# Ex10si0n/room-slam

Measured on NVIDIA B200. Metric: train traces/sec (seq500, H128) at 1/2/4/8 B200; heatmap Gpoints/s, higher is better.
Workload: dtype bf16

## Files before the change

include/roomslam_b200.h:

```cpp
#ifndef ROOMSLAM_B200_H
#define ROOMSLAM_B200_H

#include <stdint.h>

#ifdef __cplusplus
extern "C" {
#endif

const char* rs_last_error(void);
int rs_abi_version(void);
int rs_device_ok(void);
int64_t rs_launch_count(void);
int rs_set_deterministic(int on);
int rs_deterministic(void);

int rs_heatmap_bin(const float* points, int64_t n_traces, int64_t seq_len, float x_min, float y_min, float res,
                   int gx, int gy, float thr2, int32_t* occ, int32_t* stat, unsigned long long* n_dropped,
                   int accumulate, void* stream);
int rs_heatmap_bin_variant(const float* points, int64_t n_traces, int64_t seq_len, float x_min, float y_min,
                           float res, int gx, int gy, float thr2, int32_t* occ, int32_t* stat,
                           unsigned long long* n_dropped, int accumulate, int variant, void* stream);
int rs_heatmap_bin_host(const float* host_points, int64_t n_traces, int64_t seq_len, float x_min, float y_min,
                        float res, int gx, int gy, float thr2, int32_t* host_occ, int32_t* host_stat,
                        unsigned long long* host_dropped);

#define RS_GEMM_ACCUMULATE 1
#define RS_GEMM_RELU 2
#define RS_GEMM_OUT_F32 4
int rs_sgemm(const float* A, int64_t a_sm, int64_t a_sk, const float* B, int64_t b_sk, int64_t b_sn, float* C,
             int64_t ldc, const float* bias, int M, int N, int K, int flags, void* stream);
int rs_colsum_f32(const float* A, int64_t lda, int M, int N, float* out, int accumulate, void* stream);
int rs_gru_fwd_f32(const float* x, int64_t x_ld, int64_t x_rows, int64_t x_row0, int I, const float* w_ih,
                   const float* b_ih, const float* P, int64_t p_ld, int64_t p_rows, int64_t p_row0,
                   const float* w_hh_t, const float* b_hh, float* out, int64_t o_ld, int64_t o_rows, int64_t o_row0,
                   float* h_n, float* gates, const int* lengths, int B, int T, int H, void* stream);
int rs_gru_bwd_f32(const float* d_out, int64_t do_ld, int64_t do_rows, int64_t do_row0, const float* d_h_n,
                   const float* gates, const float* out, int64_t o_ld, int64_t o_rows, int64_t o_row0,
                   const float* w_hh, float* dGx, float* dGh, int64_t g_ld, int64_t g_rows, int64_t g_row0,
                   const int* lengths, int B, int T, int H, void* stream);
int rs_seq_mul_f32(const float* a, int64_t a_ld, int64_t a_rows, int64_t a_row0, const float* m, int64_t m_ld,
                   int64_t m_rows, int64_t m_row0, float* o, int64_t o_ld, int64_t o_rows, int64_t o_row0, int B, int T,
                   int C, void* stream);
int rs_heads_split_f32(const float* raw, int B, int N, int C, float* cls, float* pos, float* size, float* orient,
                       float* valid, void* stream);
int rs_heads_merge_bwd_f32(const float* raw, int B, int N, int C, const float* d_cls, const float* d_pos,
                           const float* d_size, const float* d_orient, const float* d_valid, float* d_raw, void* stream);
int rs_relu_bwd_f32(const float* dy, const float* y, float* dx, int64_t n, void* stream);
int rs_relu_bwd_bf16(const void* dy, const void* y, void* dx, int64_t n, void* stream);
int rs_loss_fwd_f32(const float* cls, const float* pos, const float* size, const float* orient, const float* vlogit,
                    const int64_t* t_cls, const float* t_pos, const float* t_size, const float* t_orient,
                    const float* t_valid, int B, int N, int C, const float* weights5, double* sums6, float* losses6,
                    float* g_cls, float* g_pos, float* g_size, float* g_orient, float* g_valid, void* stream);
int rs_loss_bwd_f32(const double* sums6, const float* d_losses6, int B, int N, int C, const float* weights5,
                    const float* g_cls, const float* g_pos, const float* g_size, const float* g_orient,
                    const float* g_valid, float* d_cls, float* d_pos, float* d_size, float* d_orient, float* d_valid,
                    void* stream);

int rs_gemm_bf16_nt(const void* A, int64_t lda, const void* B, int64_t ldb, void* C, int64_t ldc, const float* bias,
                    int64_t M, int N, int K, int flags, void* stream);
int rs_gemm_bf16_tn_acc(const void* A, int64_t lda, int64_t a_rows, int a_col0, int a_row_shift, const void* B,
                        int64_t ldb, int64_t b_rows, int b_col0, int b_row_shift, float* C, int64_t ldc, int M, int N,
                        int64_t rows, void* stream);

int rs_split_bf16x6(const float* x, int64_t ld, int64_t rows, int cols, int kpad, int role_b, void* out, int64_t ld_out,
                    void* stream);

int rs_gemm_bf16_tn_seg_acc(const void* A, int64_t lda, int64_t a_rows, int a_col0, int a_row_shift, const void* B,
                            int64_t ldb, int64_t b_rows, int b_col0, int b_row_shift, int n_seg, const int* a_seg,
                            const int* b_seg, float* C, int64_t ldc, int M, int N, int64_t rows, void* stream);

int rs_adamw_step_f32(float* p, const float* g, float* m, float* v, int64_t n, float lr, float beta1, float beta2,
                      float eps, float weight_decay, int step, float grad_scale, float max_norm, double* sumsq_scratch,
                      void* stream);

int rs_blk_gemm_nt(const void* A, int64_t a_cols, const int* a_kchunk, int k_blocks, const void* W, int n_tiles, void* C,
                   int64_t c_cols, int c_chunk0, const float* bias, int64_t n_blocks, void* stream);
int rs_blk_gemm_nt_drop(const void* A, int64_t a_cols, const int* a_kchunk, int k_blocks, const void* W, int n_tiles, void* C,
                        int64_t c_cols, int c_chunk0, int64_t n_blocks, const void* drop_bits, const float* drop_scale, int T,
                        void* stream);
int rs_blk_gemm_tn_acc(const void* A, int64_t a_cols, const int* a_mchunk, const int* c_row0, int m_tiles, const void* B,
                       int64_t b_cols, int b_chunk0, int n_cols, int b_shift, int b_broadcast, float* C, int64_t ldc,
                       int tiles, int T, void* stream);
int rs_blk_wgrad(const void* dG, int64_t a_cols, const void* ones_block, int n_roles, const int* a_mchunk,
                 const void* const* B, const int64_t* b_cols, const int* b_chunk0, const int* n_cols, const int* b_shift,
                 float* const* C, const int64_t* ldc, float* const* bias, const void* const* B2, float* const* C2,
                 int tiles, int T, void* stream);
int rs_gru_pack_weights_bf16(const float* const* w, int H, int I, int split, void* whh_img, float* b_hn, float* bias_x,
                             void* wt_proj, void* whhT_img, void* wt_dgrad, void* wih_img, void* stream);
int rs_rec_fwd_bf16(const float* x, int I, const void* P, int64_t p_cols, const void* X, const void* Wih, const void* Whh,
                    const float* b_hn, void* out,
                    void* gates, float* h_n, const int* lengths, const void* drop_bits, const float* drop_scale,
                    void* out_drop, int split, int B, int T, void* stream);
int rs_pack_x_tm(const float* x, int B, int T, int I, void* out, void* stream);
int rs_rec_bwd_bf16(const void* d_out, const float* d_h_n, const void* gates, const void* out, const void* WhhT,
                    const void* Whh, int whh_chunks, const float* b_hn, void* dG, const int* lengths, const void* drop_bits,
                    const float* drop_scale, int split, int B, int T, void* stream);
int rs_rec_fwd_bf16_wide(const float* x, int I, const void* P, const void* Wst, const float* b_hn, void* out, void* gates,
                         float* h_n, const int* lengths, const void* drop_bits, const float* drop_scale, void* out_drop,
                         int B, int T, void* stream);
int rs_rec_bwd_bf16_wide(const void* d_out, const float* d_h_n, const void* gates, const void* out, const void* WTst, void* dG,
                         const int* lengths, const void* drop_bits, const float* drop_scale, int B, int T, void* stream);
int rs_pack_drop_mask(const float* mask, int B, int T, int C, void* bits, float* scale, void* stream);
int rs_gen_drop_bits(void* bits, int B, int T, int C, float keep, uint64_t seed, float* scale, void* stream);

int rs_trace_features(const float* pts, const int64_t* offsets, int B, int max_len, int out_len, float* feats,
                      unsigned char* mask, int64_t* lengths, int* unsorted_flag, void* stream);

int rs_resample_windows_f64(const double* pts, const int64_t* offsets, const int64_t* win_trace, const int64_t* win_start,
                            int64_t n_windows, int seq_len, double step, float* out, void* stream);

int rs_lstm_fwd_f32(const float* P, int64_t p_ld, int64_t p_rows, int64_t p_row0, const float* w_hh, const float* w_hh_t,
                    float* out, int64_t o_ld, int64_t o_rows, int64_t o_row0, float* saved, int B, int T, int H,
                    void* stream);
int rs_lstm_bwd_f32(const float* d_out, int64_t do_ld, int64_t do_rows, int64_t do_row0, const float* saved,
                    const float* w_hh, float* dG, int64_t g_ld, int64_t g_rows, int64_t g_row0, int B, int T, int H,
                    void* stream);
int rs_trace_stats_f32(const float* traces, int F, const unsigned char* mask, int B, int N, float* mean, float* rms,
                       float* count, void* stream);
int64_t rs_query_attn_workspace(int B, int Q, int D, int splits);
int rs_query_attn_fwd_f32(const float* memory, int64_t m_ld, int64_t m_rows, int64_t m_row0, const float* traces, int F,
                          const unsigned char* mask, const float* mean, const float* rms, const float* qk, const float* qb,
                          int B, int N, int Q, int D, int splits, float* workspace, float* ctx, float* anchor,
                          float* summary, float* stats, void* stream);
int rs_query_attn_bwd_f32(const float* memory, int64_t m_ld, int64_t m_rows, int64_t m_row0, const float* traces, int F,
                          const unsigned char* mask, const float* mean, const float* rms, const float* count,
                          const float* qk, const float* qb, const float* ctx, const float* anchor, const float* stats,
                          const float* d_ctx, const float* d_anchor, const float* d_summary, int B, int N, int Q, int D,
                          int splits, float* d_memory, int64_t dm_ld, int64_t dm_rows, int64_t dm_row0, float* dq_part,
                          void* stream);

int rs_hungarian_match(const float* pred_boxes, const float* pred_logits, const float* gt_boxes, const int64_t* gt_labels,
                       const unsigned char* gt_valid, int B, int Q, int M, float w_class, float w_box, int* match_pred,
                       int* match_slot, int* match_rank, int* n_match, void* stream);
int rs_set_loss_f32(const float* pred_boxes, const float* pred_logits, const float* gt_boxes, const int64_t* gt_labels, int B,
                    int Q, int M, const int* match_pred, const int* match_slot, const int* n_match, float w_class, float w_l1,
                    float w_giou, float* workspace, float* losses, float* g_logits, float* g_l1, float* g_giou, void* stream);

int rs_eval_pairs(const float* pred_boxes, const float* pred_logits, const float* gt_boxes, const int64_t* gt_labels,
                  const unsigned char* gt_valid, int B, int Q, int M, const int* match_pred, const int* match_slot,
                  const int* n_match, float iou_thresh, double* workspace, double* counts, void* stream);
int rs_nms_3d(const float* pred_boxes, const float* pred_logits, int B, int Q, float conf_thr, float nms_thr, int* keep_idx,
              int* n_keep, float* conf, int* label, void* stream);
int rs_ap_flags(const float* pred_boxes, const float* pred_logits, const float* gt_boxes, const int64_t* gt_labels,
                const unsigned char* gt_valid, int B, int Q, int M, float iou_thr, int* flags, float* conf, int* label, int* n_gt,
                void* stream);

int rs_slot_eval(const float* class_logits, const float* positions, const float* sizes, const float* validity_logits,
                 const int64_t* t_classes, const float* t_positions, const float* t_sizes, const float* t_valid,
                 int64_t n_slots, int C, float iou_thr, float* conf, int* label, int* flag, int* n_gt, double* workspace,
                 double* counts, void* stream);

#ifdef __cplusplus
}
#endif
#endif
```

roomslam_b200/csrc/gemm_blk.cu:

```cuda
#include <stdlib.h>

#include "common.cuh"
#include "../../include/roomslam_b200.h"

namespace {

constexpr int CHUNK_BYTES = 2048;
constexpr int PIECE_BYTES = 8 * CHUNK_BYTES;
constexpr int NT_STAGES_MAX = 6;
constexpr int NT_MAX_KB = 24;
constexpr int NUM_THREADS = 192;

struct NtParams {
    const uint8_t* A;  long long a_block_bytes;  int a_kchunk[NT_MAX_KB];
    const uint8_t* W;
    uint8_t* C;        long long c_block_bytes;  int c_chunk0;
    const float* bias;
    int n_blocks, n_tiles, k_blocks;
    const uint8_t* drop_bits; const float* drop_scale; int drop_T; int drop_row_bytes;
};

constexpr int NT_THREADS = 320;
constexpr int NT_MAX_N = 1024;

// ... 69 lines not shown
                for (int kb = 0; kb < p.k_blocks; ++kb) {
                    rs::mbar_wait(&full_bar[stage], phase);
                    rs::tc_fence_after();
                    if (rs::elect_one()) {
                        const uint32_t ss = rs::smem_u32(stages + stage * kStageBytes);
                        const uint32_t sa = kResident ? rs::smem_u32(a_res + (ab * 4 + kb) * PIECE_BYTES) : ss;
                        const uint32_t sb = kResident ? ss : ss + PIECE_BYTES;
#pragma unroll
                        for (int k = 0; k < 4; ++k) {
                            const uint64_t da = rs::umma_desc_noswz(sa + k * 2 * CHUNK_BYTES, CHUNK_BYTES, 128);
                            const uint64_t db = rs::umma_desc_noswz(sb + k * 2 * CHUNK_BYTES, CHUNK_BYTES, 128);
                            rs::tc_mma_bf16(tmem_d, da, db, idesc, (kb | k) != 0);
                        }
                        rs::tc_commit(&empty_bar[stage]);
                        if (kb == p.k_blocks - 1) {
                            rs::tc_commit(&acc_full[acc]);
                            if (kResident && n == p.n_tiles - 1) rs::tc_commit(&a_empty[ab]);
                        }
                    }
                    __syncwarp();
                    if (++stage == NT_STAGES) { stage = 0; phase ^= 1; }
                }
                if (++acc == 2) { acc = 0; acc_phase ^= 1; }
            }
            if (kResident && ++ab == 2) { ab = 0; a_phase ^= 1; }
        }
    } else {
        const int q = warp & 3, row = q * 32 + lane;
        const int chalf = (warp - 2) >> 2;
        int acc = 0; uint32_t acc_phase = 0;
        const float dscale = p.drop_bits ? __ldg(p.drop_scale) : 1.0f;
        for (int m = blockIdx.x; m < p.n_blocks; m += gridDim.x) {
            uint8_t* cblk = p.C + (long long)m * p.c_block_bytes + row * 16;
            const uint8_t* drow = nullptr;
            if (p.drop_bits) {
                const int tp = m % (p.drop_T + 2);
                if (tp >= 1 && tp <= p.drop_T)
                    drow = p.drop_bits + (((long long)(m / (p.drop_T + 2)) * p.drop_T + (tp - 1)) * 128 + row) * p.drop_row_bytes;
            }
            for (int n = 0; n < p.n_tiles; ++n) {
                rs::mbar_wait(&acc_full[acc], acc_phase);
                rs::tc_fence_after();
                const uint32_t taddr = tmem_base + acc * 128 + chalf * 64 + (static_cast<uint32_t>(q * 32) << 16);
#pragma unroll
                for (int c0 = 0; c0 < 64; c0 += 32) {
                    uint32_t r[32];
                    rs::tmem_ld_32x32b_x32(taddr + c0, r);
                    uint32_t mbits = 0xffffffffu;
                    if (drow) mbits = __ldg(reinterpret_cast<const uint32_t*>(drow + p.c_chunk0 + n * 16 + chalf * 8 + c0 / 8));
                    rs::tmem_ld_wait();
                    if (drow) {
#pragma unroll
                        for (int e = 0; e < 32; ++e)
                            r[e] = ((mbits >> e) & 1u) ? __float_as_uint(__uint_as_float(r[e]) * dscale) : 0u;
                    }
                    const float* bs = bias_s + n * 128 + chalf * 64 + c0;
#pragma unroll
                    for (int j = 0; j < 4; ++j) {
                        uint32_t pk[4];
                        const float4 b0 = *reinterpret_cast<const float4*>(bs + 8 * j);
                        const float4 b1 = *reinterpret_cast<const float4*>(bs + 8 * j + 4);
                        const float bb[8] = {b0.x, b0.y, b0.z, b0.w, b1.x, b1.y, b1.z, b1.w};
#pragma unroll
                        for (int e = 0; e < 4; ++e) {
                            const float v0 = __uint_as_float(r[8 * j + 2 * e]) + bb[2 * e];
                            const float v1 = __uint_as_float(r[8 * j + 2 * e + 1]) + bb[2 * e + 1];
                            __nv_bfloat162 h2 = __floats2bfloat162_rn(v0, v1);
                            pk[e] = *reinterpret_cast<uint32_t*>(&h2);
                        }
                        const int chunk = p.c_chunk0 + n * 16 + chalf * 8 + c0 / 8 + j;
                        *reinterpret_cast<uint4*>(cblk + (long long)chunk * CHUNK_BYTES) = make_uint4(pk[0], pk[1], pk[2], pk[3]);
                    }
                }
                rs::tc_fence_before();
                __syncwarp();
                if (lane == 0) rs::mbar_arrive(&acc_empty[acc]);
                if (++acc == 2) { acc = 0; acc_phase ^= 1; }
            }
        }
    }
    rs::tc_fence_before();
    __syncthreads();
    if (warp == 1) rs::tmem_dealloc<256>(tmem_base);
}

constexpr int WRES_STAGES = 5;
__global__ void __launch_bounds__(NT_THREADS, 1) blk_gemm_nt_wres_kernel(const NtParams p, int n_parts) {
    extern __shared__ __align__(1024) uint8_t smem[];
    uint8_t* w_s = smem;
    uint8_t* stages = smem + p.k_blocks * 2 * PIECE_BYTES;
    float* bias_s = reinterpret_cast<float*>(stages + WRES_STAGES * PIECE_BYTES);
    uint64_t* bars = reinterpret_cast<uint64_t*>(bias_s + 256);
    uint64_t* full_bar = bars;
    uint64_t* empty_bar = bars + WRES_STAGES;
    uint64_t* acc_full = bars + 2 * WRES_STAGES;
    uint64_t* acc_empty = bars + 2 * WRES_STAGES + 2;
    uint64_t* w_full = bars + 2 * WRES_STAGES + 4;
    uint32_t* tmem_slot = reinterpret_cast<uint32_t*>(bars + 2 * WRES_STAGES + 5);
    const int warp = threadIdx.x >> 5, lane = threadIdx.x & 31;
    const int part = blockIdx.x % n_parts, group = blockIdx.x / n_parts, groups = gridDim.x / n_parts;

    if (warp == 0 && lane == 0) {
        for (int s = 0; s < WRES_STAGES; ++s) { rs::mbar_init(&full_bar[s], 1); rs::mbar_init(&empty_bar[s], 1); }
        for (int s = 0; s < 2; ++s) { rs::mbar_init(&acc_full[s], 1); rs::mbar_init(&acc_empty[s], 8); }
        rs::mbar_init(w_full, 1);
        rs::fence_mbar_init();
    }
    if (warp == 1) rs::tmem_alloc<512>(tmem_slot);
    for (int i = threadIdx.x; i < 256; i += NT_THREADS) bias_s[i] = p.bias ? p.bias[part * 256 + i] : 0.0f;
    rs::tc_fence_before();
    __syncthreads();
    rs::tc_fence_after();
    const uint32_t tmem_base = *tmem_slot;

    if (warp == 0) {
        if (rs::elect_one()) {
            rs::mbar_expect_tx(w_full, p.k_blocks * 2 * PIECE_BYTES);
            for (int kb = 0; kb < p.k_blocks; ++kb)
                for (int half = 0; half < 2; ++half) {
                    const uint8_t* src = p.W + ((long long)(part * 2 + half) * p.k_blocks + kb) * PIECE_BYTES;
                    for (int c = 0; c < 8; ++c)
                        rs::bulk_load(w_s + kb * 2 * PIECE_BYTES + c * 2 * CHUNK_BYTES + half * CHUNK_BYTES, src + c * CHUNK_BYTES,
                                      CHUNK_BYTES, w_full);
                }
            int stage = 0; uint32_t phase = 0;
            for (int m = group; m < p.n_blocks; m += groups) {
                const uint8_t* ablk = p.A + (long long)m * p.a_block_bytes;
                for (int kb = 0; kb < p.k_blocks; ++kb) {
                    rs::mbar_wait(&empty_bar[stage], phase ^ 1);
                    rs::mbar_expect_tx(&full_bar[stage], PIECE_BYTES);
                    rs::bulk_load(stages + stage * PIECE_BYTES, ablk + (long long)p.a_kchunk[kb] * CHUNK_BYTES, PIECE_BYTES, &full_bar[stage]);
                    if (++stage == WRES_STAGES) { stage = 0; phase ^= 1; }
                }
            }
        }
    } else if (warp == 1) {
        constexpr uint32_t idesc = rs::umma_idesc_bf16(128, 256, 0, 0);
        rs::mbar_wait(w_full, 0);
        rs::tc_fence_after();
        int stage = 0; uint32_t phase = 0; int acc = 0; uint32_t acc_phase = 0;
        const uint32_t w_addr = rs::smem_u32(w_s);
        for (int m = group; m < p.n_blocks; m += groups) {
            rs::mbar_wait(&acc_empty[acc], acc_phase ^ 1);
            rs::tc_fence_after();
            const uint32_t tmem_d = tmem_base + acc * 256;
            for (int kb = 0; kb < p.k_blocks; ++kb) {
                rs::mbar_wait(&full_bar[stage], phase);
                rs::tc_fence_after();
                if (rs::elect_one()) {
                    const uint32_t sa = rs::smem_u32(stages + stage * PIECE_BYTES);
                    const uint32_t sb = w_addr + kb * 2 * PIECE_BYTES;
#pragma unroll
                    for (int k = 0; k < 4; ++k) {
                        const uint64_t da = rs::umma_desc_noswz(sa + k * 2 * CHUNK_BYTES, CHUNK_BYTES, 128);
                        const uint64_t db = rs::umma_desc_noswz(sb + k * 2 * (2 * CHUNK_BYTES), 2 * CHUNK_BYTES, 128);
                        rs::tc_mma_bf16(tmem_d, da, db, idesc, (kb | k) != 0);
                    }
                    rs::tc_commit(&empty_bar[stage]);
                    if (kb == p.k_blocks - 1) rs::tc_commit(&acc_full[acc]);
                }
                __syncwarp();
                if (++stage == WRES_STAGES) { stage = 0; phase ^= 1; }
            }
            if (++acc == 2) { acc = 0; acc_phase ^= 1; }
        }
    } else {
// ... 292 lines not shown
        if (i1 > i0) acc_phase ^= 1;
        __syncthreads();
        rs::tc_fence_after();
    }
    rs::tc_fence_before();
    __syncthreads();
    if (p.paired) rs::cluster_sync_all();
    if (warp == 1) rs::tmem_dealloc<512>(tmem_base);
}

int g_sms = 0;
int num_sms() {
    if (g_sms == 0) {
        int dev = 0;
        cudaGetDevice(&dev);
        cudaDeviceGetAttribute(&g_sms, cudaDevAttrMultiProcessorCount, dev);
    }
    return g_sms;
}

}

static int blk_gemm_nt_impl(const void* A, int64_t a_cols, const int* a_kchunk, int k_blocks, const void* W,
                            int n_tiles, void* C, int64_t c_cols, int c_chunk0, const float* bias, int64_t n_blocks,
                            const void* drop_bits, const float* drop_scale, int drop_T, void* stream_) {
    cudaStream_t stream = static_cast<cudaStream_t>(stream_);
    if (rs::check_device_sm100()) return 3;
    if (n_blocks == 0) return 0;
    RS_REQUIRE(A && W && C && a_kchunk, "rs_blk_gemm_nt: null pointer");
    RS_REQUIRE(k_blocks >= 1 && k_blocks <= NT_MAX_KB && n_tiles >= 1, "rs_blk_gemm_nt: 1 <= k_blocks <= %d", NT_MAX_KB);
    RS_REQUIRE(a_cols % 8 == 0 && c_cols % 8 == 0 && n_blocks < (1ll << 31), "rs_blk_gemm_nt: bad shape");
    NtParams p = {};
    p.A = static_cast<const uint8_t*>(A); p.a_block_bytes = a_cols * 256;
    for (int i = 0; i < k_blocks; ++i) {
        RS_REQUIRE(a_kchunk[i] >= 0 && (a_kchunk[i] + 8) * 8 <= a_cols, "rs_blk_gemm_nt: K block %d outside the A block", i);
        p.a_kchunk[i] = a_kchunk[i];
    }
    RS_REQUIRE((c_chunk0 + n_tiles * 16) * 8 <= c_cols, "rs_blk_gemm_nt: output columns outside the C block");
    p.W = static_cast<const uint8_t*>(W);
    p.C = static_cast<uint8_t*>(C); p.c_block_bytes = c_cols * 256; p.c_chunk0 = c_chunk0;
    p.bias = bias; p.n_blocks = (int)n_blocks; p.n_tiles = n_tiles; p.k_blocks = k_blocks;
    RS_REQUIRE(n_tiles * 128 <= NT_MAX_N, "rs_blk_gemm_nt: at most %d output columns", NT_MAX_N);
    if (drop_bits) {
        RS_REQUIRE(drop_scale && drop_T >= 1 && n_blocks % (drop_T + 2) == 0 && c_chunk0 % 4 == 0 && c_cols % 32 == 0 && !bias,
                   "rs_blk_gemm_nt_drop: the mask needs drop_scale, whole tiles of T + 2 blocks, 32-column alignment and no bias");
        p.drop_bits = static_cast<const uint8_t*>(drop_bits); p.drop_scale = drop_scale; p.drop_T = drop_T;
        p.drop_row_bytes = (int)(c_cols / 8);
    }
    const int grid = (int)(n_blocks < num_sms() ? n_blocks : num_sms());
    static const bool wres_off = getenv("RS_NT_WRES") && atoi(getenv("RS_NT_WRES")) == 0;
    if (k_blocks <= 4 && n_tiles % 2 == 0 && n_tiles / 2 <= 8 && n_blocks >= 2 * num_sms() && !wres_off && !drop_bits) {
        const int n_parts = n_tiles / 2;
        const int groups = num_sms() / n_parts;
        const int smem = k_blocks * 2 * PIECE_BYTES + WRES_STAGES * PIECE_BYTES + 256 * 4 + 256;
        RS_CUDA_OK(cudaFuncSetAttribute(blk_gemm_nt_wres_kernel, cudaFuncAttributeMaxDynamicSharedMemorySize, smem));
        blk_gemm_nt_wres_kernel<<<groups * n_parts, NT_THREADS, smem, stream>>>(p, n_parts);
        rs::count_launch();
    } else if (k_blocks <= 4) {
        const int smem = 2 * 4 * PIECE_BYTES + 5 * PIECE_BYTES + NT_MAX_N * 4 + 256;
        RS_CUDA_OK(cudaFuncSetAttribute(blk_gemm_nt_kernel<true>, cudaFuncAttributeMaxDynamicSharedMemorySize, smem));
        blk_gemm_nt_kernel<true><<<grid, NT_THREADS, smem, stream>>>(p);
        rs::count_launch();
    } else {
        const int smem = 6 * 2 * PIECE_BYTES + NT_MAX_N * 4 + 256;
        RS_CUDA_OK(cudaFuncSetAttribute(blk_gemm_nt_kernel<false>, cudaFuncAttributeMaxDynamicSharedMemorySize, smem));
        blk_gemm_nt_kernel<false><<<grid, NT_THREADS, smem, stream>>>(p);
        rs::count_launch();
    }
    RS_CUDA_OK(cudaGetLastError());
    return 0;
}

extern "C" int rs_blk_gemm_nt(const void* A, int64_t a_cols, const int* a_kchunk, int k_blocks, const void* W,
                              int n_tiles, void* C, int64_t c_cols, int c_chunk0, const float* bias, int64_t n_blocks,
                              void* stream_) {
    return blk_gemm_nt_impl(A, a_cols, a_kchunk, k_blocks, W, n_tiles, C, c_cols, c_chunk0, bias, n_blocks, nullptr, nullptr, 0, stream_);
}

extern "C" int rs_blk_gemm_nt_drop(const void* A, int64_t a_cols, const int* a_kchunk, int k_blocks, const void* W,
                                   int n_tiles, void* C, int64_t c_cols, int c_chunk0, int64_t n_blocks, const void* drop_bits,
                                   const float* drop_scale, int T, void* stream_) {
    RS_REQUIRE(drop_bits != nullptr, "rs_blk_gemm_nt_drop: drop_bits is required");
    return blk_gemm_nt_impl(A, a_cols, a_kchunk, k_blocks, W, n_tiles, C, c_cols, c_chunk0, nullptr, n_blocks, drop_bits, drop_scale, T, stream_);
}

extern "C" int rs_blk_gemm_tn_acc(const void* A, int64_t a_cols, const int* a_mchunk, const int* c_row0, int m_tiles,
                                  const void* B, int64_t b_cols, int b_chunk0, int n_cols, int b_shift, int b_broadcast,
                                  float* C, int64_t ldc, int tiles, int T, void* stream_) {
    cudaStream_t stream = static_cast<cudaStream_t>(stream_);
    if (rs::check_device_sm100()) return 3;
    RS_REQUIRE(A && B && C && a_mchunk && c_row0, "rs_blk_gemm_tn_acc: null pointer");
    RS_REQUIRE(m_tiles >= 1 && m_tiles <= TN_MAX_MT, "rs_blk_gemm_tn_acc: 1 <= m_tiles <= %d", TN_MAX_MT);
    RS_REQUIRE(n_cols >= 16 && n_cols <= 256 && n_cols % 16 == 0, "rs_blk_gemm_tn_acc: n_cols must be a multiple of 16 in [16,256]");
    RS_REQUIRE(b_shift >= -1 && b_shift <= 1 && tiles >= 0 && T >= 0, "rs_blk_gemm_tn_acc: bad arguments");
    RS_REQUIRE((b_chunk0 * 8 + n_cols) <= b_cols && a_cols % 8 == 0 && b_cols % 8 == 0, "rs_blk_gemm_tn_acc: B columns outside the block");
    const long long total = (long long)tiles * T;
    if (total == 0) return 0;
    RS_REQUIRE(total < (1ll << 31), "rs_blk_gemm_tn_acc: too many blocks");
    TnParams p = {};
    p.A = static_cast<const uint8_t*>(A); p.a_block_bytes = a_cols * 256;
    for (int i = 0; i < m_tiles; ++i) {
        RS_REQUIRE(a_mchunk[i] >= 0 && (a_mchunk[i] + 16) * 8 <= a_cols, "rs_blk_gemm_tn_acc: M tile %d outside the A block", i);
        p.a_mchunk[i] = a_mchunk[i]; p.c_row0[i] = c_row0[i];
    }
    p.B = static_cast<const uint8_t*>(B); p.b_block_bytes = b_broadcast ? 0 : b_cols * 256; p.b_chunk0 = b_chunk0; p.n_cols = n_cols; p.b_shift = b_shift;
    p.C = C; p.ldc = ldc; p.m_tiles = m_tiles; p.tiles = tiles; p.T = T; p.Tp = T + 2;
    const bool det = rs::deterministic();
    int splits = (det ? rs::kDetSplitSms : num_sms()) / m_tiles;
    if (splits < 1) splits = 1;
    if (splits > total) splits = (int)total;
    p.blocks_per_split = (int)((total + splits - 1) / splits);
    p.splits = (int)((total + p.blocks_per_split - 1) / p.blocks_per_split);
    const int smem = 2 * (2 * PIECE_BYTES + n_cols * 256) + 256;
    const int items = p.m_tiles * p.splits;
    const int grid = items < num_sms() ? items : num_sms();
    if (det) {
        rs::StreamScratch ws(stream);
        const long long slot = (long long)m_tiles * 128 * n_cols;
        RS_CUDA_OK(ws.alloc(sizeof(float) * p.splits * slot));
        p.C = ws.as<float>(); p.ldc = n_cols;
        RS_CUDA_OK(cudaFuncSetAttribute(blk_gemm_tn_kernel<true>, cudaFuncAttributeMaxDynamicSharedMemorySize, smem));
        blk_gemm_tn_kernel<true><<<grid, NUM_THREADS, smem, stream>>>(p);
        rs::count_launch();
        RS_CUDA_OK(cudaGetLastError());
        rs::SlotSum<float> jobs[TN_MAX_MT];
        for (int i = 0; i < m_tiles; ++i) jobs[i] = {ws.as<float>() + (long long)i * 128 * n_cols, C + (long long)c_row0[i] * ldc, ldc, 128, n_cols};
        return rs::slot_sum(jobs, m_tiles, p.splits, slot, true, stream);
    }
    RS_CUDA_OK(cudaFuncSetAttribute(blk_gemm_tn_kernel<false>, cudaFuncAttributeMaxDynamicSharedMemorySize, smem));
    blk_gemm_tn_kernel<false><<<grid, NUM_THREADS, smem, stream>>>(p);
    rs::count_launch();
    RS_CUDA_OK(cudaGetLastError());
    return 0;
}

extern "C" int rs_blk_wgrad(const void* dG, int64_t a_cols, const void* ones_block, int n_roles, const int* a_mchunk,
                            const void* const* B, const int64_t* b_cols, const int* b_chunk0, const int* n_cols,
                            const int* b_shift, float* const* C, const int64_t* ldc, float* const* bias,
                            const void* const* B2, float* const* C2, int tiles, int T, void* stream_) {
    cudaStream_t stream = static_cast<cudaStream_t>(stream_);
    if (rs::check_device_sm100()) return 3;
    RS_REQUIRE(dG && ones_block && a_mchunk && B && b_cols && b_chunk0 && n_cols && b_shift && C && ldc && bias && B2 && C2,
               "rs_blk_wgrad: null pointer");
    RS_REQUIRE(n_roles >= 1 && n_roles <= WG_MAX_ROLES, "rs_blk_wgrad: 1 <= n_roles <= %d", WG_MAX_ROLES);
    const long long total = (long long)tiles * T;
    if (total == 0) return 0;
    RS_REQUIRE(total < (1ll << 31) && a_cols % 8 == 0, "rs_blk_wgrad: bad shape");
    WgParams p = {};
    p.A = static_cast<const uint8_t*>(dG); p.a_block_bytes = a_cols * 256;
    p.ones = static_cast<const uint8_t*>(ones_block);
    p.n_roles = n_roles; p.tiles = tiles; p.T = T; p.Tp = T + 2;
    int max_n = 16;
    for (int r = 0; r < n_roles; ++r) {
        RS_REQUIRE(a_mchunk[r] >= 0 && (a_mchunk[r] + 16) * 8 <= a_cols, "rs_blk_wgrad: role %d columns outside dG", r);
        RS_REQUIRE(n_cols[r] >= 0 && n_cols[r] <= 256 && n_cols[r] % 16 == 0, "rs_blk_wgrad: role %d n_cols", r);
        RS_REQUIRE(n_cols[r] == 0 || (b_chunk0[r] * 8 + n_cols[r] <= b_cols[r] && B[r] && C[r]), "rs_blk_wgrad: role %d B/C", r);
        RS_REQUIRE(n_cols[r] > 0 || B2[r] || bias[r], "rs_blk_wgrad: role %d has nothing to do", r);
        RS_REQUIRE(!B2[r] || C2[r], "rs_blk_wgrad: role %d has B2 but no C2", r);
        RS_REQUIRE(b_shift[r] >= -1 && b_shift[r] <= 1, "rs_blk_wgrad: role %d shift", r);
        WgRole& R = p.role[r];
        R.a_mchunk = a_mchunk[r]; R.B = static_cast<const uint8_t*>(B[r]); R.b_block_bytes = b_cols[r] * 256;
        R.b_chunk0 = b_chunk0[r]; R.n_cols = n_cols[r]; R.b_shift = b_shift[r]; R.C = C[r]; R.ldc = ldc[r]; R.bias = bias[r];
        R.B2 = static_cast<const uint8_t*>(B2[r]); R.b2_block_bytes = 16 * 256; R.C2 = C2[r]; R.ldc2 = 16;
        if (n_cols[r] > max_n) max_n = n_cols[r];
    }
    p.max_b_bytes = max_n * 256;
// ... 55 lines not shown
```

roomslam_b200/functional_bf16.py:

```python
from __future__ import annotations

import ctypes
import os
from typing import Optional

import torch

from . import _lib
from . import functional as F_
from . import layout as L
from .functional import _need_cuda, _p, _stream, ktime

H = 128

MAX_X_INPUTS = 16


def x_col(i: int, k: int) -> int:
    return 3 * i + k if i < 2 else 8 + 3 * (i - 2) + k


def x_steps(I: int) -> int:
    return (3 * I + 2 + 15) // 16

# ... 139 lines not shown
                with ktime("rec_fwd_pair_kernel", rec_flops + 2.0 * B * T * 6 * H * Il):
                    _lib.call("rs_rec_fwd_bf16", 0, 0, 0, 0, _p(X), _p(wih_img), _p(whh_img), _p(b_hn), _p(out), _p(gates), _p(h_n),
                              _p(lengths), _p(d_bits), _p(d_scale), _p(out_drop), 0, B, T, st)
                saved_in = X
            else:
                X = xin
                P = torch.empty(tiles, T + 2, 6 * H // 8, L.TILE, 8, device=dev, dtype=torch.bfloat16)
                with ktime("blk_gemm_nt_kernel(projection)", 2.0 * tiles * L.TILE * (T + 2) * 6 * H * Il):
                    _nt(X, Il, [8 * k for k in range(Il // 64)] * (1 + split), wt, 6, P, 6 * H, 0, bias_x.reshape(-1).contiguous(),
                        tiles * (T + 2), st)
                with ktime("rec_fwd_pair_kernel", rec_flops):
                    _lib.call("rs_rec_fwd_bf16", 0, 0, _p(P), 6 * H, 0, 0, _p(whh_img), _p(b_hn), _p(out), _p(gates), _p(h_n), _p(lengths),
                              _p(d_bits), _p(d_scale), _p(out_drop), split, B, T, st)
                del P
                saved_in = X
        ctx.meta = (padded_in, B, T, Il, split)
        ctx.drop = drop
        ctx.lengths = lengths
        ctx.save_for_backward(out, gates, saved_in, whhT_img, wt_dgrad, whh_img, b_hn)
        if out_drop is not None:
            return out_drop, h_n
        return out, h_n

    @staticmethod
    @_lib.on_tensor_device
    def backward(ctx, d_out, d_h_n):
        padded_in, B, T, Il, split = ctx.meta
        out, gates, saved_in, whhT_img, wt_dgrad, whh_img, b_hn = ctx.saved_tensors
        if gates is None:
            raise RuntimeError("GRULayerBF16Fn: forward ran without saving activations (nothing required grad)")
        dev = out.device
        st = torch.cuda.current_stream(dev).cuda_stream
        tiles = L.n_tiles(B)
        with torch.no_grad():
            d_out = d_out.contiguous().to(torch.bfloat16) if d_out is not None else None
            d_h_n = d_h_n.contiguous().float() if d_h_n is not None else None
            dG = torch.empty(tiles, T + 2, 8 * H // 8, L.TILE, 8, device=dev, dtype=torch.bfloat16)
            with ktime("rec_bwd_pair_kernel", 2.0 * B * T * 2 * 3 * H * H):
                d_bits, d_scale = ctx.drop if (ctx.drop is not None and ctx.mask_d_out) else (None, None)
                _lib.call("rs_rec_bwd_bf16", _p(d_out), _p(d_h_n), _p(gates), _p(out), _p(whhT_img), _p(whh_img), whh_img.shape[1],
                          _p(b_hn), _p(dG), _p(ctx.lengths), _p(d_bits), _p(d_scale), split, B, T, st)
            dW_ih, dW_hh, db_ih, db_hh, d_xin = grads_from_dG_128(dG, out, saved_in, padded_in, B, T, Il, split, wt_dgrad,
                                                                  ctx.in_drop, padded_in and ctx.needs_input_grad[0])
            dW_ih = dW_ih[:, :Il].contiguous() if not padded_in else dW_ih
        return (d_xin, None, None, dW_ih[:3 * H], dW_hh[0], db_ih[0], db_hh[0], dW_ih[3 * H:], dW_hh[1], db_ih[1], db_hh[1])


def grads_from_dG_128(dG, out, saved_in, padded_in, B, T, Il, split, wt_dgrad, in_drop, need_dx):
    dev = dG.device
    st = torch.cuda.current_stream(dev).cuda_stream
    tiles = L.n_tiles(B)
    dW_hh = torch.zeros(2, 3 * H, H, device=dev)
    sums = torch.zeros(2, 4, H, device=dev)
    roles = []
    if not padded_in:
        xa_tm = torch.empty(tiles, T + 2, 2, L.TILE, 8, device=dev, dtype=torch.bfloat16)
        _lib.call("rs_pack_x_tm", _p(saved_in), B, T, Il, _p(xa_tm), st)
        dW_ih_buf = torch.zeros(6 * H, 16, device=dev)
        for d in (0, 1):
            sh = -1 if d == 0 else 1
            for g in (0, 1):
                roles.append((d * 64 + g * 16, out, 2 * H, d * 16, H, sh, dW_hh[d, g * H:], H, sums[d, g],
                              xa_tm, dW_ih_buf[(d * 3 + g) * H:]))
            roles.append((d * 64 + 48, out, 2 * H, d * 16, H, sh, dW_hh[d, 2 * H:], H, sums[d, 3], None, None))
            roles.append((d * 64 + 32, None, 0, 0, 0, 0, None, 0, sums[d, 2], xa_tm, dW_ih_buf[(d * 3 + 2) * H:]))
        flops = 2.0 * tiles * L.TILE * T * (6 * H * 16 + 6 * H * H + 8 * H * 16)
    else:
        dW_ih_buf = torch.zeros(6 * H, Il, device=dev)
        for d in (0, 1):
            sh = -1 if d == 0 else 1
            ih = lambda g: (d * 64 + g * 16, saved_in, Il, 0, Il, 0, dW_ih_buf[(d * 3 + g) * H:], Il, sums[d, g], None, None)
            hh = lambda gi, g: (d * 64 + g * 16, out, 2 * H, d * 16, H, sh, dW_hh[d, gi * H:], H,
                                sums[d, 3] if g == 3 else None, None, None)
            roles += [ih(0), hh(0, 0), ih(1), hh(1, 1), ih(2), hh(2, 3)]
        flops = 2.0 * tiles * L.TILE * T * (6 * H * Il + 6 * H * H + 8 * H * 16)
    with ktime("blk_wgrad_kernel", flops):
        _wgrad(dG, 8 * H, _ones_block(dev), roles, tiles, T, st)
    db_ih = sums[:, :3].reshape(2, 3 * H)
    db_hh = torch.cat([sums[:, :2].reshape(2, 2 * H), sums[:, 3]], 1)
    dX = None
    if need_dx:
        dX = torch.empty(tiles, T + 2, Il // 8, L.TILE, 8, device=dev, dtype=torch.bfloat16)
        kch = [d * 64 + g * 16 + hf * 8 for d in (0, 1) for g in (0, 1, 2) for hf in (0, 1)]
        with ktime("blk_gemm_nt_kernel(dgrad)", 2.0 * tiles * L.TILE * (T + 2) * 6 * H * Il):
            _nt(dG, 8 * H, kch * (1 + split), wt_dgrad, Il // 128, dX, Il, 0, None, tiles * (T + 2), st, in_drop, T)
    return dW_ih_buf, dW_hh, db_ih, db_hh, dX


def wide_fwd_image(w_ih, w_hh, b_ih, b_hh, w_ih_r, w_hh_r, b_ih_r, b_hh_r, layer0: bool):
    HW = w_hh.shape[1]
    dev, bf = w_hh.device, torch.bfloat16
    Il = w_ih.shape[1]
    half = torch.ones(3 * HW, device=dev)
    half[:2 * HW] = 0.5
    w_hh_cat = torch.stack([w_hh, w_hh_r], 0).float()
    w_ih_cat = torch.cat([w_ih, w_ih_r], 0).float()
    b_hn = torch.stack([b_hh[2 * HW:], b_hh_r[2 * HW:]], 0).float().contiguous()
    bias_x = torch.stack([b_ih, b_ih_r], 0).float().clone()
    bias_x[0, :2 * HW] += b_hh[:2 * HW]
    bias_x[1, :2 * HW] += b_hh_r[:2 * HW]
    bias_x *= half[None, :]
    whs = w_hh_cat * half[None, :, None]
    w_ih_fwd = (w_ih_cat.view(2, 3 * HW, Il) * half[None, :, None])
    rows = lambda t, r: torch.cat([t[:, g * HW + 128 * r: g * HW + 128 * r + 128] for g in range(3)], 1)
    per_rank = []
    for r in (0, 1):
        img = rows(whs, r).view(2, 384, HW // 16, 2, 8).permute(0, 2, 3, 1, 4)
        if layer0:
            xs = x_steps(Il)
            w_hi = w_ih_fwd.to(bf).float()
            b_hi = bias_x.to(bf).float()
            xcols = torch.zeros(2, 3 * HW, 16 * xs, device=dev)
            for c in range(Il):
                xcols[:, :, x_col(c, 0)] = w_hi[:, :, c]
                xcols[:, :, x_col(c, 1)] = w_hi[:, :, c]
                xcols[:, :, x_col(c, 2)] = w_ih_fwd[:, :, c] - w_hi[:, :, c]
            xcols[:, :, 6] = b_hi
            xcols[:, :, 7] = bias_x - b_hi
            xstep = rows(xcols, r).view(2, 384, xs, 2, 8).permute(0, 2, 3, 1, 4)
            pad = torch.zeros(2, xs % 2, 2, 384, 8, device=dev)
            img = torch.cat([img, xstep, pad], 1)
        per_rank.append(img)
    wst = torch.stack(per_rank, 1).to(bf).contiguous()
    return wst, b_hn, bias_x, w_ih_fwd, w_ih_cat, w_hh_cat


def wide_bwd_image(w_hh_cat):
    HW = w_hh_cat.shape[2]
    whhT = w_hh_cat.transpose(1, 2)
    return torch.stack([whhT[:, 128 * r: 128 * r + 128].reshape(2, 128, 3 * HW // 16, 2, 8).permute(0, 2, 3, 1, 4)
                        for r in (0, 1)], 1).to(torch.bfloat16).contiguous()


class GRULayerBF16WideFn(torch.autograd.Function):

    HW = 256

    @staticmethod
    @_lib.on_tensor_device
    def forward(ctx, xin, meta, mask, w_ih, w_hh, b_ih, b_hh, w_ih_r, w_hh_r, b_ih_r, b_hh_r):
        ctx.set_materialize_grads(False)
        _need_cuda(xin, w_ih, w_hh)
        HW = GRULayerBF16WideFn.HW
        padded_in, B, T = meta[:3]
        lengths = meta[3] if len(meta) > 3 else None
        drop = meta[4] if len(meta) > 4 else None
        ctx.in_drop = meta[6] if len(meta) > 6 else None
        ctx.mask_d_out = bool(meta[7]) if len(meta) > 7 else False
        if mask is not None:
            raise _lib.RoomSlamError("GRULayerBF16WideFn: pass dropout as packed bits on the producing layer (meta[4])")
        if w_hh.shape[1] != HW:
            raise _lib.RoomSlamError(f"GRULayerBF16WideFn is built for hidden_size = {HW}")
        dev, st, bf = xin.device, _stream(xin), torch.bfloat16
        need_grad = any(ctx.needs_input_grad)
        tiles, Il = L.n_tiles(B), w_ih.shape[1]
        with torch.no_grad():
            if not padded_in:
                _check_x_inputs(Il)
            wst, b_hn, bias_x, w_ih_fwd, w_ih_cat, w_hh_cat = wide_fwd_image(w_ih, w_hh, b_ih, b_hh, w_ih_r, w_hh_r, b_ih_r, b_hh_r,
                                                                             not padded_in)
            out = L.empty_tm(B, T, 2 * HW, dev, zero_pads=False)
            out_drop = L.empty_tm(B, T, 2 * HW, dev, zero_pads=False) if drop is not None else None
            d_bits, d_scale = drop if drop is not None else (None, None)
            h_n = torch.empty(2, B, HW, device=dev)
            gates = torch.empty(tiles, T, 2, 4 * HW // 8, L.TILE, 8, device=dev, dtype=bf) if need_grad else None
            rec_flops = 2.0 * B * T * 2 * 3 * HW * HW
            if not padded_in:
                x = xin.contiguous().float()
# ... 205 lines not shown
```

Baseline: 422,600.

## Add cluster-pair dgrad kernel multicasting weight tiles for input-gradient GEMM

```diff
diff --git a/include/roomslam_b200.h b/include/roomslam_b200.h
--- a/include/roomslam_b200.h
+++ b/include/roomslam_b200.h
@@ -78,6 +78,8 @@
 int rs_blk_gemm_nt_drop(const void* A, int64_t a_cols, const int* a_kchunk, int k_blocks, const void* W, int n_tiles, void* C,
                         int64_t c_cols, int c_chunk0, int64_t n_blocks, const void* drop_bits, const float* drop_scale, int T,
                         void* stream);
+int rs_blk_dgrad_pair(const void* dG, int64_t a_cols, const int* a_kchunk, int k_blocks, const void* W, void* C,
+                      int64_t n_blocks, const void* drop_bits, const float* drop_scale, int T, void* stream);
 int rs_blk_gemm_tn_acc(const void* A, int64_t a_cols, const int* a_mchunk, const int* c_row0, int m_tiles, const void* B,
                        int64_t b_cols, int b_chunk0, int n_cols, int b_shift, int b_broadcast, float* C, int64_t ldc,
                        int tiles, int T, void* stream);
diff --git a/roomslam_b200/csrc/gemm_blk.cu b/roomslam_b200/csrc/gemm_blk.cu
--- a/roomslam_b200/csrc/gemm_blk.cu
+++ b/roomslam_b200/csrc/gemm_blk.cu
@@ -175,6 +175,134 @@
     rs::tc_fence_before();
     __syncthreads();
     if (warp == 1) rs::tmem_dealloc<256>(tmem_base);
+}
+
+constexpr int DP_STAGES = 4;
+constexpr int DP_STAGE_BYTES = 3 * PIECE_BYTES;
+template <bool kDrop>
+__global__ void __launch_bounds__(NT_THREADS, 1) blk_dgrad_pair_kernel(const NtParams p) {
+    extern __shared__ __align__(1024) uint8_t smem[];
+    uint8_t* stages = smem;
+    uint64_t* bars = reinterpret_cast<uint64_t*>(smem + DP_STAGES * DP_STAGE_BYTES);
+    uint64_t* full_bar = bars;
+    uint64_t* empty_bar = bars + DP_STAGES;
+    uint64_t* acc_full = bars + 2 * DP_STAGES;
+    uint64_t* acc_empty = bars + 2 * DP_STAGES + 2;
+    uint32_t* tmem_slot = reinterpret_cast<uint32_t*>(bars + 2 * DP_STAGES + 4);
+    const int warp = threadIdx.x >> 5, lane = threadIdx.x & 31;
+    const int crank = static_cast<int>(rs::cluster_ctarank());
+    const int pair = blockIdx.x >> 1, n_pairs = gridDim.x >> 1;
+    const int pair_blocks = (p.n_blocks + 1) >> 1;
+    auto block_of = [&](int j) { return min(2 * j + crank, p.n_blocks - 1); };
+
+    if (warp == 0 && lane == 0) {
+        for (int s = 0; s < DP_STAGES; ++s) { rs::mbar_init(&full_bar[s], 1); rs::mbar_init(&empty_bar[s], 2); }
+        for (int s = 0; s < 2; ++s) { rs::mbar_init(&acc_full[s], 1); rs::mbar_init(&acc_empty[s], 8); }
+        rs::fence_mbar_init();
+    }
+    if (warp == 1) rs::tmem_alloc<512>(tmem_slot);
+    rs::tc_fence_before();
+    __syncthreads();
+    rs::cluster_sync_all();
+    rs::tc_fence_after();
+    const uint32_t tmem_base = *tmem_slot;
+
+    if (warp == 0) {
+        if (rs::elect_one()) {
+            int stage = 0; uint32_t phase = 0;
+            for (int j = pair; j < pair_blocks; j += n_pairs) {
+                const uint8_t* ablk = p.A + (long long)block_of(j) * p.a_block_bytes;
+                for (int kb = 0; kb < p.k_blocks; ++kb) {
+                    rs::mbar_wait(&empty_bar[stage], phase ^ 1);
+                    uint8_t* ss = stages + stage * DP_STAGE_BYTES;
+                    rs::mbar_expect_tx(&full_bar[stage], DP_STAGE_BYTES);
+                    rs::bulk_load(ss, ablk + (long long)p.a_kchunk[kb] * CHUNK_BYTES, PIECE_BYTES, &full_bar[stage]);
+                    rs::bulk_load_mc(ss + (1 + crank) * PIECE_BYTES, p.W + ((long long)crank * p.k_blocks + kb) * PIECE_BYTES,
+                                     PIECE_BYTES, &full_bar[stage], 3);
+                    if (++stage == DP_STAGES) { stage = 0; phase ^= 1; }
+                }
+            }
+        }
+    } else if (warp == 1) {
+        constexpr uint32_t idesc = rs::umma_idesc_bf16(128, 128, 0, 0);
+        int stage = 0; uint32_t phase = 0; int acc = 0; uint32_t acc_phase = 0;
+        for (int j = pair; j < pair_blocks; j += n_pairs) {
+            rs::mbar_wait(&acc_empty[acc], acc_phase ^ 1);
+            rs::tc_fence_after();
+            const uint32_t tmem_d = tmem_base + acc * 256;
+            for (int kb = 0; kb < p.k_blocks; ++kb) {
+                rs::mbar_wait(&full_bar[stage], phase);
+                rs::tc_fence_after();
+                if (rs::elect_one()) {
+                    const uint32_t sa = rs::smem_u32(stages + stage * DP_STAGE_BYTES);
+#pragma unroll
+                    for (int n = 0; n < 2; ++n)
+#pragma unroll
+                        for (int k = 0; k < 4; ++k) {
+                            const uint64_t da = rs::umma_desc_noswz(sa + k * 2 * CHUNK_BYTES, CHUNK_BYTES, 128);
+                            const uint64_t db = rs::umma_desc_noswz(sa + (1 + n) * PIECE_BYTES + k * 2 * CHUNK_BYTES, CHUNK_BYTES, 128);
+                            rs::tc_mma_bf16(tmem_d + n * 128, da, db, idesc, (kb | k) != 0);
+                        }
+                    rs::tc_commit_mc(&empty_bar[stage], 3);
+                    if (kb == p.k_blocks - 1) rs::tc_commit(&acc_full[acc]);
+                }
+                __syncwarp();
+                if (++stage == DP_STAGES) { stage = 0; phase ^= 1; }
+            }
+            if (++acc == 2) { acc = 0; acc_phase ^= 1; }
+        }
+    } else {
+        const int q = warp & 3, row = q * 32 + lane;
+        const int n = (warp - 2) >> 2;
+        int acc = 0; uint32_t acc_phase = 0;
+        const float dscale = kDrop ? __ldg(p.drop_scale) : 1.0f;
+        for (int j = pair; j < pair_blocks; j += n_pairs) {
+            const int m = block_of(j);
+            uint8_t* cblk = p.C + (long long)m * p.c_block_bytes + row * 16;
+            const uint8_t* drow = nullptr;
+            if (kDrop) {
+                const int tp = m % (p.drop_T + 2);
+                if (tp >= 1 && tp <= p.drop_T)
+                    drow = p.drop_bits + (((long long)(m / (p.drop_T + 2)) * p.drop_T + (tp - 1)) * 128 + row) * p.drop_row_bytes;
+            }
+            rs::mbar_wait(&acc_full[acc], acc_phase);
+            rs::tc_fence_after();
+            const uint32_t taddr = tmem_base + acc * 256 + n * 128 + (static_cast<uint32_t>(q * 32) << 16);
+#pragma unroll
+            for (int c0 = 0; c0 < 128; c0 += 32) {
+                uint32_t r[32];
+                rs::tmem_ld_32x32b_x32(taddr + c0, r);
+                uint32_t mbits = 0xffffffffu;
+                if (kDrop && drow) mbits = __ldg(reinterpret_cast<const uint32_t*>(drow + n * 16 + c0 / 8));
+                rs::tmem_ld_wait();
+                if (kDrop && drow) {
+#pragma unroll
+                    for (int e = 0; e < 32; ++e)
+                        r[e] = ((mbits >> e) & 1u) ? __float_as_uint(__uint_as_float(r[e]) * dscale) : 0u;
+                }
+#pragma unroll
+                for (int jj = 0; jj < 4; ++jj) {
+                    uint32_t pk[4];
+#pragma unroll
+                    for (int e = 0; e < 4; ++e) {
+                        __nv_bfloat162 h2 = __floats2bfloat162_rn(__uint_as_float(r[8 * jj + 2 * e]) + 0.0f,
+                                                                  __uint_as_float(r[8 * jj + 2 * e + 1]) + 0.0f);
+                        pk[e] = *reinterpret_cast<uint32_t*>(&h2);
+                    }
+                    const int chunk = n * 16 + c0 / 8 + jj;
+                    *reinterpret_cast<uint4*>(cblk + (long long)chunk * CHUNK_BYTES) = make_uint4(pk[0], pk[1], pk[2], pk[3]);
+                }
+            }
+            rs::tc_fence_before();
+            __syncwarp();
+            if (lane == 0) rs::mbar_arrive(&acc_empty[acc]);
+            if (++acc == 2) { acc = 0; acc_phase ^= 1; }
+        }
+    }
+    rs::tc_fence_before();
+    __syncthreads();
+    rs::cluster_sync_all();
+    if (warp == 1) rs::tmem_dealloc<512>(tmem_base);
 }
 
 constexpr int WRES_STAGES = 5;
@@ -633,6 +761,45 @@
                                    const float* drop_scale, int T, void* stream_) {
     RS_REQUIRE(drop_bits != nullptr, "rs_blk_gemm_nt_drop: drop_bits is required");
     return blk_gemm_nt_impl(A, a_cols, a_kchunk, k_blocks, W, n_tiles, C, c_cols, c_chunk0, nullptr, n_blocks, drop_bits, drop_scale, T, stream_);
+}
+
+extern "C" int rs_blk_dgrad_pair(const void* dG, int64_t a_cols, const int* a_kchunk, int k_blocks, const void* W, void* C,
+                                 int64_t n_blocks, const void* drop_bits, const float* drop_scale, int T, void* stream_) {
+    cudaStream_t stream = static_cast<cudaStream_t>(stream_);
+    if (rs::check_device_sm100()) return 3;
+    if (n_blocks == 0) return 0;
+    RS_REQUIRE(dG && W && C && a_kchunk, "rs_blk_dgrad_pair: null pointer");
+    RS_REQUIRE(k_blocks >= 1 && k_blocks <= NT_MAX_KB, "rs_blk_dgrad_pair: 1 <= k_blocks <= %d", NT_MAX_KB);
+    RS_REQUIRE(a_cols % 8 == 0 && n_blocks < (1ll << 31), "rs_blk_dgrad_pair: bad shape");
+    NtParams p = {};
+    p.A = static_cast<const uint8_t*>(dG); p.a_block_bytes = a_cols * 256;
+    for (int i = 0; i < k_blocks; ++i) {
+        RS_REQUIRE(a_kchunk[i] >= 0 && (a_kchunk[i] + 8) * 8 <= a_cols, "rs_blk_dgrad_pair: K block %d outside the dG block", i);
+        p.a_kchunk[i] = a_kchunk[i];
+    }
+    p.W = static_cast<const uint8_t*>(W);
+    p.C = static_cast<uint8_t*>(C); p.c_block_bytes = 256 * 256;
+    p.n_blocks = (int)n_blocks; p.n_tiles = 2; p.k_blocks = k_blocks;
+    if (drop_bits) {
+        RS_REQUIRE(drop_scale && T >= 1 && n_blocks % (T + 2) == 0,
+                   "rs_blk_dgrad_pair: the mask needs drop_scale and whole tiles of T + 2 blocks");
+        p.drop_bits = static_cast<const uint8_t*>(drop_bits); p.drop_scale = drop_scale; p.drop_T = T; p.drop_row_bytes = 256 / 8;
+    }
+    const long long pair_blocks = (n_blocks + 1) / 2;
+    const int pairs = (int)(pair_blocks < num_sms() / 2 ? pair_blocks : num_sms() / 2);
+    const int smem = DP_STAGES * DP_STAGE_BYTES + 256;
+    const auto kernel = drop_bits ? blk_dgrad_pair_kernel<true> : blk_dgrad_pair_kernel<false>;
+    RS_CUDA_OK(cudaFuncSetAttribute(kernel, cudaFuncAttributeMaxDynamicSharedMemorySize, smem));
+    cudaLaunchConfig_t cfg = {};
+    cfg.gridDim = dim3(2 * pairs); cfg.blockDim = dim3(NT_THREADS); cfg.dynamicSmemBytes = smem; cfg.stream = stream;
+    cudaLaunchAttribute attr[1];
+    attr[0].id = cudaLaunchAttributeClusterDimension;
+    attr[0].val.clusterDim.x = 2; attr[0].val.clusterDim.y = 1; attr[0].val.clusterDim.z = 1;
+    cfg.attrs = attr; cfg.numAttrs = 1;
+    RS_CUDA_OK(cudaLaunchKernelEx(&cfg, kernel, p));
+    rs::count_launch();
+    RS_CUDA_OK(cudaGetLastError());
+    return 0;
 }
 
 extern "C" int rs_blk_gemm_tn_acc(const void* A, int64_t a_cols, const int* a_mchunk, const int* c_row0, int m_tiles,
diff --git a/roomslam_b200/functional_bf16.py b/roomslam_b200/functional_bf16.py
--- a/roomslam_b200/functional_bf16.py
+++ b/roomslam_b200/functional_bf16.py
@@ -245,8 +245,16 @@
     if need_dx:
         dX = torch.empty(tiles, T + 2, Il // 8, L.TILE, 8, device=dev, dtype=torch.bfloat16)
         kch = [d * 64 + g * 16 + hf * 8 for d in (0, 1) for g in (0, 1, 2) for hf in (0, 1)]
-        with ktime("blk_gemm_nt_kernel(dgrad)", 2.0 * tiles * L.TILE * (T + 2) * 6 * H * Il):
-            _nt(dG, 8 * H, kch * (1 + split), wt_dgrad, Il // 128, dX, Il, 0, None, tiles * (T + 2), st, in_drop, T)
+        flops = 2.0 * tiles * L.TILE * (T + 2) * 6 * H * Il
+        if Il == 2 * H and not split:
+            d_bits, d_scale = in_drop if in_drop is not None else (None, None)
+            kc = L.int_array(kch)
+            with ktime("blk_dgrad_pair_kernel", flops):
+                _lib.call("rs_blk_dgrad_pair", _p(dG), 8 * H, ctypes.addressof(kc), len(kch), _p(wt_dgrad), _p(dX),
+                          tiles * (T + 2), _p(d_bits), _p(d_scale), T, st)
+        else:
+            with ktime("blk_gemm_nt_kernel(dgrad)", flops):
+                _nt(dG, 8 * H, kch * (1 + split), wt_dgrad, Il // 128, dX, Il, 0, None, tiles * (T + 2), st, in_drop, T)
     return dW_ih_buf, dW_hh, db_ih, db_hh, dX
 
 
```

New measurement: 428,100, median of 6. +1.3%, better.
